# cmavro/GNN-RAG

Measured on NVIDIA H100. Metric: questions/sec (GNN forward+score) on WebQSP-shape subgraphs; agg-kernel HBM GB/s, higher is better.
Workload: dtype f32

## Files before the change

### gnn_rag_b200/csrc/linear_tc.cu

```cuda
#include "wgmma.cuh"

namespace gr {

int g_tc_cluster = 1;
int g_tc_bk = 32;
int g_tc_tma_store = 1;

namespace {

using namespace tc;
constexpr int kThreads = 384;
constexpr int kConsumerWarps = 8;
constexpr int kLaunchRegs = 168, kProducerRegs = 40, kConsumerRegs = 232;
static_assert(128 * kProducerRegs + 256 * kConsumerRegs <= kThreads * kLaunchRegs, "register budget");

__global__ void split_bf16_seg_kernel(const float* __restrict__ W, int64_t ldw, int64_t N, int64_t Kpad,
                                      int seg, int pitch, __nv_bfloat16* __restrict__ hi,
                                      __nv_bfloat16* __restrict__ lo, int64_t ldo) {
  const int64_t total = N * Kpad;
  const int64_t stride = (int64_t)gridDim.x * blockDim.x;
  for (int64_t i = (int64_t)blockIdx.x * blockDim.x + threadIdx.x; i < total; i += stride) {
    const int64_t n = i / Kpad, k = i - n * Kpad;
    const int sidx = (int)(k / pitch), c = (int)(k - (int64_t)sidx * pitch);
    float v = c < seg ? __ldg(W + n * ldw + (int64_t)sidx * seg + c) : 0.f;
    const __nv_bfloat16 h = __float2bfloat16_rn(v);
    hi[n * ldo + k] = h;
    lo[n * ldo + k] = __float2bfloat16_rn(v - __bfloat162float(h));
  }
}

__global__ void split_bf16_kernel(const float* __restrict__ A, int64_t lda, int64_t M, int64_t K,
                                  __nv_bfloat16* __restrict__ hi, __nv_bfloat16* __restrict__ lo,
                                  int64_t ldo, int vec_ok, int vec_st) {
  const int64_t kq = (K + 3) / 4;
  const int64_t total = M * kq;
  const int64_t stride = (int64_t)gridDim.x * blockDim.x;
  for (int64_t i = (int64_t)blockIdx.x * blockDim.x + threadIdx.x; i < total; i += stride) {
    const int64_t m = i / kq, k = (i - m * kq) * 4;
    float v[4] = {0.f, 0.f, 0.f, 0.f};
    const float* src = A + m * lda + k;
    if (vec_ok && k + 3 < K) {
      float4 t = __ldg(reinterpret_cast<const float4*>(src));
      v[0] = t.x; v[1] = t.y; v[2] = t.z; v[3] = t.w;
    } else {
#pragma unroll
      for (int q = 0; q < 4; ++q)
        if (k + q < K) v[q] = __ldg(src + q);
    }
    __nv_bfloat16 h[4], l[4];
#pragma unroll
    for (int q = 0; q < 4; ++q) {
      h[q] = __float2bfloat16_rn(v[q]);
      l[q] = __float2bfloat16_rn(v[q] - __bfloat162float(h[q]));
    }
    __nv_bfloat16* ph = hi + m * ldo + k;
    __nv_bfloat16* pl = lo + m * ldo + k;
    if (vec_st && k + 3 < ldo) {
      *reinterpret_cast<uint2*>(ph) = *reinterpret_cast<uint2*>(h);
      *reinterpret_cast<uint2*>(pl) = *reinterpret_cast<uint2*>(l);
    } else {
#pragma unroll
      for (int q = 0; q < 4; ++q)
        if (k + q < ldo) { ph[q] = h[q]; pl[q] = l[q]; }
    }
  }
}

struct TcParams {
  const float* bias;
  float* C;
  int64_t ldc;
  __nv_bfloat16* c_hi;
  __nv_bfloat16* c_lo;
  int64_t ldc16;
  const float* w_score;
  float* dots;
  int M, N, K, n_pad, n16, stages, num_tiles;
  uint32_t flags;
  int tma_store;
  int kg_T, kg_G, kg_pitch, kg_nkb, kg_one0, kg_one1, kg_nb0;
};

template <int NP, int CS, int BK, bool GROUPED>
__global__ void __launch_bounds__(kThreads, 1)
linear_tc_kernel(const __grid_constant__ CUtensorMap map_a_hi, const __grid_constant__ CUtensorMap map_a_lo,
                 const __grid_constant__ CUtensorMap map_w_hi, const __grid_constant__ CUtensorMap map_w_lo,
                 const __grid_constant__ CUtensorMap map_c, const __grid_constant__ CUtensorMap map_c_hi,
                 const __grid_constant__ CUtensorMap map_c_lo, const TcParams p) {
  extern __shared__ __align__(1024) uint8_t smem_raw[];
  uint8_t* smem = reinterpret_cast<uint8_t*>((reinterpret_cast<uintptr_t>(smem_raw) + 1023) & ~(uintptr_t)1023);
  const int a_bytes = BM * BK * 2;
  constexpr int w_bytes = NP * BK * 2;
  const bool single = (p.flags & GR_LINEAR_BF16_SINGLE) != 0;
  const int w_off = single ? a_bytes : 2 * a_bytes;
  const int stage_bytes = single ? a_bytes + w_bytes : 2 * a_bytes + 2 * w_bytes;
  uint8_t* s_out = smem + (size_t)p.stages * stage_bytes;
  uint64_t* bars = reinterpret_cast<uint64_t*>(s_out + 2 * kStageOutBytes);
  uint64_t* full_bar = bars;
  uint64_t* empty_bar = bars + p.stages;
  float* s_bias = reinterpret_cast<float*>(bars + 2 * p.stages);
  float* s_ws = s_bias + 256;
  for (int i = threadIdx.x; i < 256; i += kThreads) {
    s_bias[i] = (p.bias && i < p.N) ? p.bias[i] : 0.f;
    s_ws[i] = (p.w_score && i < p.N) ? p.w_score[i] : 0.f;
  }

  const int warp = threadIdx.x >> 5, lane = threadIdx.x & 31;
  const int nkb = GROUPED ? p.kg_nkb : (p.K + BK - 1) / BK;
  const int crank = CS > 1 ? (int)cluster_ctarank() : 0;
  const int ncluster = gridDim.x / CS, cid = blockIdx.x / CS;
  const int ngroups = (p.num_tiles + CS - 1) / CS;
  constexpr uint16_t kMask = (uint16_t)((1u << CS) - 1);

  if (threadIdx.x == 0) {
    for (int s = 0; s < p.stages; ++s) {
      mbar_init(&full_bar[s], 1);
      mbar_init(&empty_bar[s], kConsumerWarps * CS);
    }
    asm volatile("fence.mbarrier_init.release.cluster;" ::: "memory");
  }
  __syncthreads();
  if (CS > 1) cluster_sync_all();

  if (warp < 4) {
    asm volatile("setmaxnreg.dec.sync.aligned.u32 %0;" ::"n"(kProducerRegs));
    if (warp == 0 && lane == 0) {
      uint32_t phase = 0;
      int s = 0;
      constexpr int w_rows = NP / CS;
      const int w_slice = w_rows * BK * 2;
      for (int g = cid; g < ngroups; g += ncluster) {
        const int m0 = (g * CS + crank) * BM;
        for (int kb = 0; kb < nkb; ++kb) {
          mbar_wait(&empty_bar[s], phase ^ 1);
          uint8_t* st = smem + (size_t)s * stage_bytes;
          mbar_expect_tx(&full_bar[s], (uint32_t)stage_bytes);
          int a_col = kb * BK;
          if constexpr (GROUPED) {
            if (p.kg_nb0 == 0) {
              const int g = kb / p.kg_T, t = kb - g * p.kg_T, ni = p.kg_T >> 1;
              const int seg = t == 0 ? 0 : 1 + 2 * ((t - 1) % ni) + (t - 1) / ni;
              a_col = seg * p.kg_pitch + g * BK;
            } else {
              const int g = min(kb / p.kg_T, p.kg_G), t = kb - g * p.kg_T;
              a_col = t == 0 ? g * BK : p.kg_nb0 + (kb - g - 1) * BK;
            }
          }
          tma_load_2d(st, &map_a_hi, &full_bar[s], a_col, m0);
          if (!single) tma_load_2d(st + a_bytes, &map_a_lo, &full_bar[s], a_col, m0);
          if (CS == 1) {
            tma_load_2d(st + w_off, &map_w_hi, &full_bar[s], kb * BK, 0);
            if (!single) tma_load_2d(st + w_off + w_bytes, &map_w_lo, &full_bar[s], kb * BK, 0);
          } else {
            tma_load_2d_mc(st + w_off + crank * w_slice, &map_w_hi, &full_bar[s], kb * BK,
                           crank * w_rows, kMask);
            if (!single)
              tma_load_2d_mc(st + w_off + w_bytes + crank * w_slice, &map_w_lo, &full_bar[s], kb * BK,
                             crank * w_rows, kMask);
          }
          if (++s == p.stages) { s = 0; phase ^= 1; }
        }
      }
    }
  } else {
    asm volatile("setmaxnreg.inc.sync.aligned.u32 %0;" ::"n"(kConsumerRegs));
    const int cw = (warp - 4) >> 2, wq = warp & 3;
    const EpiOut e{s_bias, s_ws, (p.flags & GR_LINEAR_RELU) != 0};
    const int r = wq * 16 + (lane >> 2), cq = lane & 3;
    uint8_t* stg = s_out + (size_t)cw * kStageOutBytes;
    const bool issuer = wq == 0 && lane == 0;
    const bool vec_c = p.C && (p.ldc % 2 == 0) && ((reinterpret_cast<uintptr_t>(p.C) & 7) == 0);
    const bool vec_h = p.c_hi && (p.ldc16 % 2 == 0) && ((reinterpret_cast<uintptr_t>(p.c_hi) & 3) == 0) &&
                       ((reinterpret_cast<uintptr_t>(p.c_lo) & 3) == 0);
    uint32_t phase = 0;
    int s = 0;
    for (int g = cid; g < ngroups; g += ncluster) {
      const int tile = g * CS + crank;
      float acc[NP / 2];
#pragma unroll
      for (int i = 0; i < NP / 2; ++i) acc[i] = 0.f;
      int prev = -1;
      for (int kb = 0; kb < nkb; ++kb) {
        mbar_wait(&full_bar[s], phase);
        const uint32_t sa = smem_u32(smem + (size_t)s * stage_bytes);
        const uint32_t a_row = (uint32_t)(cw * WG_M * BK * 2);
        const uint64_t da_hi = make_smem_desc<BK>(sa + a_row), da_lo = make_smem_desc<BK>(sa + a_bytes + a_row);
        const uint64_t dw_hi = make_smem_desc<BK>(sa + w_off), dw_lo = make_smem_desc<BK>(sa + w_off + w_bytes);
        if constexpr (GROUPED) {
          if (kb >= p.kg_one0 && kb < p.kg_one1) mma_kblock<NP, BK, 1, false>(acc, da_hi, da_lo, dw_hi, dw_lo);
          else mma_kblock<NP, BK, BK / MMA_K, false>(acc, da_hi, da_lo, dw_hi, dw_lo);
        } else if (single) {
          mma_kblock<NP, BK, BK / MMA_K, true>(acc, da_hi, da_lo, dw_hi, dw_lo);
        } else {
          mma_kblock<NP, BK, BK / MMA_K, false>(acc, da_hi, da_lo, dw_hi, dw_lo);
        }
        wgmma_wait<1>();
        if (prev >= 0 && lane == 0) release_slot<CS>(&empty_bar[prev]);
        prev = s;
        if (++s == p.stages) { s = 0; phase ^= 1; }
      }
      wgmma_wait<0>();
      if (prev >= 0 && lane == 0) release_slot<CS>(&empty_bar[prev]);

      const int64_t row0 = (int64_t)tile * BM + cw * WG_M + r;
      float dot0 = 0.f, dot1 = 0.f;
#pragma unroll
      for (int q = 0; q < NP / 16; ++q) {
        const int c0 = 16 * q;
        if (c0 >= p.n_pad) continue;
        float v[8];
        epi_values(acc, q, cq, e, v, dot0, dot1);
        if (p.tma_store) {
          epi_store_tma(v, stg, r, cq, issuer, 1 + cw, &map_c, &map_c_hi, &map_c_lo, p.C != nullptr,
                        p.c_hi != nullptr, c0, tile * BM + cw * WG_M);
          continue;
        }
#pragma unroll
        for (int b = 0; b < 2; ++b) {
          const int col = c0 + 8 * b + 2 * cq;
#pragma unroll
          for (int hr = 0; hr < 2; ++hr) {
            const int64_t row = row0 + 8 * hr;
            if (row >= p.M) continue;
            const float x0 = v[4 * b + 2 * hr], x1 = v[4 * b + 2 * hr + 1];
            if (p.C) {
              float* c = p.C + row * p.ldc + col;
              if (vec_c && col + 1 < p.N) {
                *reinterpret_cast<float2*>(c) = make_float2(x0, x1);
              } else {
                if (col < p.N) c[0] = x0;
                if (col + 1 < p.N) c[1] = x1;
              }
            }
            if (p.c_hi) {
              uint32_t lo;
              const uint32_t hi = split_hi_lo(x0, x1, lo);
              unsigned short* ph = reinterpret_cast<unsigned short*>(p.c_hi + row * p.ldc16 + col);
              unsigned short* pl = reinterpret_cast<unsigned short*>(p.c_lo + row * p.ldc16 + col);
              if (vec_h && col + 1 < p.n16) {
                *reinterpret_cast<uint32_t*>(ph) = hi;
                *reinterpret_cast<uint32_t*>(pl) = lo;
              } else {
                if (col < p.n16) { ph[0] = (unsigned short)(hi & 0xFFFF); pl[0] = (unsigned short)(lo & 0xFFFF); }
                if (col + 1 < p.n16) { ph[1] = (unsigned short)(hi >> 16); pl[1] = (unsigned short)(lo >> 16); }
              }
            }
          }
        }
      }
      epi_dots(dot0, dot1, p.dots, row0, p.M, cq);
    }
    if (p.tma_store && issuer) asm volatile("cp.async.bulk.wait_group 0;" ::: "memory");
  }
  __syncthreads();
  if (CS > 1) cluster_sync_all();
}

struct TcPlan {
  int64_t kp;
  int n_pad, np, stages, bk;
  size_t a_plane_bytes, w_plane_bytes, total_bytes, w_only_bytes, smem_bytes;
  bool ok;
};

TcPlan plan_tc(int64_t M, int64_t N, int64_t K, bool single = false) {
  TcPlan t{};
  const int BK = g_tc_bk == 64 ? 64 : 32;
  t.ok = (N >= 8 && N <= 256 && K >= 8 && M >= 1);
  t.kp = (K + 7) / 8 * 8;
  t.n_pad = (int)((N + 15) / 16 * 16);
  t.np = t.n_pad <= 64 ? 64 : t.n_pad <= 128 ? 128 : t.n_pad <= 208 ? 208 : 256;
  const size_t stage = (single ? 1 : 2) * ((size_t)BM * BK * 2 + (size_t)t.np * BK * 2);
  int stages = (int)((227 * 1024 - 1024 - 2048 - 128 - 2 * kStageOutBytes) / stage);
  t.stages = stages > 8 ? 8 : stages;
  if (t.stages < 2) t.ok = false;
  t.bk = BK;
  t.smem_bytes = (size_t)t.stages * stage + 1024  + 2 * t.stages * 8 + 2 * 256 * 4 + 2 * kStageOutBytes;
  t.a_plane_bytes = align_up((size_t)M * t.kp * 2, 256);
  t.w_plane_bytes = align_up((size_t)N * t.kp * 2, 256);
  t.total_bytes = 2 * t.a_plane_bytes + 2 * t.w_plane_bytes;
  t.w_only_bytes = 2 * t.w_plane_bytes;
  return t;
}


int split_launch(const float* A, int64_t lda, int64_t M, int64_t K, __nv_bfloat16* hi, __nv_bfloat16* lo,
                 int64_t ldo, cudaStream_t stream) {
  int va = (lda % 4 == 0) && ((reinterpret_cast<uintptr_t>(A) & 15) == 0);
  int64_t work = M * ((K + 3) / 4);
  int grid = (int)std::min<int64_t>(ceil_div(work, 256), 32LL * sm_count());
  int vs = (ldo % 4 == 0) && ((reinterpret_cast<uintptr_t>(hi) & 7) == 0) &&
           ((reinterpret_cast<uintptr_t>(lo) & 7) == 0);
  split_bf16_kernel<<<grid, 256, 0, stream>>>(A, lda, M, K, hi, lo, ldo, va, vs);
  GR_CHECK_LAUNCH();
  return GR_OK;
}

template <int NP, int CS, int BK, bool GROUPED = false>
int launch_tc_cs(const CUtensorMap& m_a_hi, const CUtensorMap& m_a_lo, const CUtensorMap& m_w_hi,
                 const CUtensorMap& m_w_lo, const CUtensorMap& m_c, const CUtensorMap& m_c_hi,
                 const CUtensorMap& m_c_lo, const TcPlan& t, const TcParams& p, cudaStream_t stream) {
  const int ngroups = (p.num_tiles + CS - 1) / CS;
  const int nclusters = std::max(1, std::min(ngroups, sm_count() / CS));
  return launch_cluster<linear_tc_kernel<NP, CS, BK, GROUPED>>("gr_linear_tc", kLaunchRegs, CS, nclusters * CS, kThreads,
                                                               t.smem_bytes, stream, m_a_hi, m_a_lo, m_w_hi, m_w_lo,
                                                               m_c, m_c_hi, m_c_lo, p);
}

template <int NP>
int launch_tc_np(const CUtensorMap* const (&m)[7], int cs, const TcPlan& t, const TcParams& p, cudaStream_t stream) {
  if (p.kg_T) {
    if (cs == 2) return launch_tc_cs<NP, 2, 32, true>(*m[0], *m[1], *m[2], *m[3], *m[4], *m[5], *m[6], t, p, stream);
    return launch_tc_cs<NP, 1, 32, true>(*m[0], *m[1], *m[2], *m[3], *m[4], *m[5], *m[6], t, p, stream);
  }
  if (t.bk == 64) {
    if (cs == 2) return launch_tc_cs<NP, 2, 64>(*m[0], *m[1], *m[2], *m[3], *m[4], *m[5], *m[6], t, p, stream);
    return launch_tc_cs<NP, 1, 64>(*m[0], *m[1], *m[2], *m[3], *m[4], *m[5], *m[6], t, p, stream);
  }
  if (cs == 2) return launch_tc_cs<NP, 2, 32>(*m[0], *m[1], *m[2], *m[3], *m[4], *m[5], *m[6], t, p, stream);
  return launch_tc_cs<NP, 1, 32>(*m[0], *m[1], *m[2], *m[3], *m[4], *m[5], *m[6], t, p, stream);
}

int launch_tc(const __nv_bfloat16* a_hi, const __nv_bfloat16* a_lo, int64_t lda16,
              const __nv_bfloat16* w_hi, const __nv_bfloat16* w_lo, int64_t ldw16, const TcPlan& t,
              TcParams p, cudaStream_t stream) {
  p.n_pad = t.n_pad; p.stages = t.stages;
  p.num_tiles = (int)ceil_div(p.M, BM);
  int cs = (g_tc_cluster >= 2 && (t.np / 2) % 8 == 0 && p.num_tiles >= 2) ? 2 : 1;
  CUtensorMap m_a_hi, m_a_lo, m_w_hi, m_w_lo;
  const int64_t w_cols = p.kg_T ? ldw16 : p.K;
  const int64_t a_cols = p.kg_nb0 ? p.kg_nb0 + (int64_t)(p.kg_T - 1) * p.kg_pitch : p.K;
  if (!make_tmap(&m_a_hi, a_hi, p.M, a_cols, lda16, BM, t.bk) || !make_tmap(&m_a_lo, a_lo, p.M, a_cols, lda16, BM, t.bk) ||
      !make_tmap(&m_w_hi, w_hi, p.N, w_cols, ldw16, t.np / cs, t.bk) ||
      !make_tmap(&m_w_lo, w_lo, p.N, w_cols, ldw16, t.np / cs, t.bk)) {
    set_error("gr_linear_tc: cuTensorMapEncodeTiled failed (pointers must be 16-byte aligned, row strides "
              "multiples of 8 elements)");
    return GR_ERR_CUDA;
  }
  p.n16 = (int)std::min<int64_t>((p.N + 15) / 16 * 16, p.ldc16);
  CUtensorMap m_c, m_c_hi, m_c_lo;
  memset(&m_c, 0, sizeof(m_c)); memset(&m_c_hi, 0, sizeof(m_c_hi)); memset(&m_c_lo, 0, sizeof(m_c_lo));
  bool ok = g_tc_tma_store != 0;
  if (ok && p.C) ok = p.N % 4 == 0 && make_out_tmap(&m_c, p.C, p.M, p.N, p.ldc, 4);
  if (ok && p.c_hi) ok = make_out_tmap(&m_c_hi, p.c_hi, p.M, p.n16, p.ldc16, 2) &&
                         make_out_tmap(&m_c_lo, p.c_lo, p.M, p.n16, p.ldc16, 2);
  p.tma_store = ok ? 1 : 0;
  const CUtensorMap* m[7] = {&m_a_hi, &m_a_lo, &m_w_hi, &m_w_lo, &m_c, &m_c_hi, &m_c_lo};
  switch (t.np) {
    case 64: return launch_tc_np<64>(m, cs, t, p, stream);
    case 128: return launch_tc_np<128>(m, cs, t, p, stream);
    case 208: return launch_tc_np<208>(m, cs, t, p, stream);
    default: return launch_tc_np<256>(m, cs, t, p, stream);
  }
}

}

bool linear_tc_supported(int64_t M, int64_t N, int64_t K) {
  return plan_tc(M, N, K).ok && get_encode_fn() != nullptr;
}

}

extern "C" size_t gr_linear_tc_workspace_bytes(int64_t M, int64_t N, int64_t K) {
  if (M <= 0 || N <= 0 || K <= 0) return 0;
  return gr::plan_tc(M, N, K).total_bytes;
}

extern "C" size_t gr_linear_tc_planes_workspace_bytes(int64_t N, int64_t K) {
  if (N <= 0 || K <= 0) return 0;
  return gr::plan_tc(1, N, K).w_only_bytes;
}

extern "C" int gr_split_bf16(const float* A, int64_t lda, int64_t M, int64_t K, void* hi, void* lo,
                             int64_t ld_out, void* stream_) {
  using namespace gr;
  GR_CHECK_ARG(A && hi && lo, "null pointer");
  GR_CHECK_ARG(M > 0 && K > 0 && lda >= K && ld_out >= K && ld_out % 8 == 0, "bad shape / ld_out % 8 != 0");
  return split_launch(A, lda, M, K, reinterpret_cast<__nv_bfloat16*>(hi), reinterpret_cast<__nv_bfloat16*>(lo),
                      ld_out, reinterpret_cast<cudaStream_t>(stream_));
}

extern "C" int gr_linear_tc(const float* A, int64_t lda, const float* W, int64_t ldw, const float* bias,
                            float* C, int64_t ldc, int64_t M, int64_t N, int64_t K, uint32_t flags,
                            void* workspace, size_t workspace_bytes, void* stream_) {
  using namespace gr;
  cudaStream_t stream = reinterpret_cast<cudaStream_t>(stream_);
  GR_CHECK_ARG(A && W && C && workspace, "null pointer");
  GR_CHECK_ARG(M > 0 && N > 0 && K > 0, "M, N, K must be positive");
  GR_CHECK_ARG(lda >= K && ldw >= K && ldc >= N, "leading dimension smaller than row length");
  GR_CHECK_ARG(M < (int64_t)0x7fffffff - BM, "M exceeds int32 range");
  TcPlan t = plan_tc(M, N, K);
  if (!t.ok) {
    set_error("gr_linear_tc: unsupported shape M=%lld N=%lld K=%lld (need 8 <= N <= 256, K >= 8)",
              (long long)M, (long long)N, (long long)K);
    return GR_ERR_UNSUPPORTED;
  }
  if (int rc = check_workspace(__func__, workspace, workspace_bytes, t.total_bytes)) return rc;
  if ((reinterpret_cast<uintptr_t>(workspace) & 255) != 0) {
    set_error("gr_linear_tc: workspace must be 256-byte aligned");
    return GR_ERR_INVALID_ARG;
  }
  char* ws = reinterpret_cast<char*>(workspace);
  __nv_bfloat16* a_hi = reinterpret_cast<__nv_bfloat16*>(ws);
  __nv_bfloat16* a_lo = reinterpret_cast<__nv_bfloat16*>(ws + t.a_plane_bytes);
  __nv_bfloat16* w_hi = reinterpret_cast<__nv_bfloat16*>(ws + 2 * t.a_plane_bytes);
  __nv_bfloat16* w_lo = reinterpret_cast<__nv_bfloat16*>(ws + 2 * t.a_plane_bytes + t.w_plane_bytes);
  int rc = split_launch(A, lda, M, K, a_hi, a_lo, t.kp, stream);
  if (rc != GR_OK) return rc;
  rc = split_launch(W, ldw, N, K, w_hi, w_lo, t.kp, stream);
  if (rc != GR_OK) return rc;
  TcParams p{};
  p.bias = bias; p.C = C; p.ldc = ldc;
  p.M = (int)M; p.N = (int)N; p.K = (int)K; p.flags = flags;
  return launch_tc(a_hi, a_lo, t.kp, w_hi, w_lo, t.kp, t, p, stream);
}

extern "C" int gr_linear_tc_planes(const void* A_hi, const void* A_lo, int64_t lda16, const float* W,
                                   int64_t ldw, const float* bias, float* C, int64_t ldc, void* C_hi,
                                   void* C_lo, int64_t ldc16, const float* w_score, float* dots, int64_t M,
                                   int64_t N, int64_t K, int64_t k_seg, int64_t k_seg_pitch, uint32_t flags,
                                   void* workspace, size_t workspace_bytes, void* stream_) {
  using namespace gr;
  cudaStream_t stream = reinterpret_cast<cudaStream_t>(stream_);
  GR_CHECK_ARG(A_hi && (A_lo || (flags & GR_LINEAR_BF16_SINGLE)) && W && workspace, "null pointer");
  GR_CHECK_ARG(C || C_hi, "no output requested");
  GR_CHECK_ARG(M > 0 && N > 0 && K > 0, "M, N, K must be positive");
  const bool grouped = (flags & GR_LINEAR_K_GROUPED) != 0;
  const bool korder = (flags & GR_LINEAR_K_ORDER_PLANES) != 0;
  GR_CHECK_ARG(!korder || grouped, "GR_LINEAR_K_ORDER_PLANES modifies GR_LINEAR_K_GROUPED and needs it");
  if (grouped) {
    GR_CHECK_ARG(k_seg > 0 && k_seg_pitch >= k_seg && k_seg_pitch % 16 == 0,
                 "GR_LINEAR_K_GROUPED needs segmented K: k_seg > 0 and k_seg_pitch >= k_seg, a multiple of 16");
    GR_CHECK_ARG(K % k_seg_pitch == 0 && (K / k_seg_pitch) % 2 == 1,
                 "GR_LINEAR_K_GROUPED needs an odd number of segments (2 I + 1)");
    GR_CHECK_ARG(g_tc_bk != 64, "GR_LINEAR_K_GROUPED needs 32-column k-blocks (tc_bk = 32)");
    GR_CHECK_ARG(!(flags & GR_LINEAR_BF16_SINGLE), "GR_LINEAR_K_GROUPED does not combine with GR_LINEAR_BF16_SINGLE");
  }
  const bool segmented = grouped || (k_seg > 0 && k_seg_pitch > k_seg);
  GR_CHECK_ARG(lda16 >= K && lda16 % 8 == 0, "lda16 must be >= K and a multiple of 8");
  GR_CHECK_ARG(!segmented || K % k_seg_pitch == 0, "K must be a multiple of k_seg_pitch");
  GR_CHECK_ARG(ldw >= (segmented ? K / k_seg_pitch * k_seg : K), "ldw smaller than the weight row length");
  GR_CHECK_ARG(!C || ldc >= N, "ldc smaller than N");
  GR_CHECK_ARG(!C_hi || (C_lo && ldc16 >= N), "C_lo missing or ldc16 smaller than N");
  GR_CHECK_ARG(!dots || w_score, "dots requested without w_score");
  GR_CHECK_ARG(M < (int64_t)0x7fffffff - BM, "M exceeds int32 range");
  TcPlan t = plan_tc(M, N, K, (flags & GR_LINEAR_BF16_SINGLE) != 0);
  if (!t.ok) {
    set_error("gr_linear_tc_planes: unsupported shape M=%lld N=%lld K=%lld", (long long)M, (long long)N,
              (long long)K);
    return GR_ERR_UNSUPPORTED;
  }
  const int num_ins = grouped ? (int)(K / k_seg_pitch / 2) : 0;
  const GroupedK gk = grouped ? plan_grouped_k(k_seg_pitch, num_ins, N, korder) : GroupedK{};
  const int64_t nb0 = (k_seg_pitch + 31) / 32 * 32;
  GR_CHECK_ARG(!korder || lda16 >= nb0 + 2 * num_ins * k_seg_pitch,
               "GR_LINEAR_K_ORDER_PLANES: lda16 must cover the neighbour region (round32(k_seg_pitch) + (K - k_seg_pitch) "
               "columns)");
  const size_t w_plane_bytes = grouped ? gk.w_plane_bytes : t.w_plane_bytes;
  if (workspace_bytes < 2 * w_plane_bytes || (reinterpret_cast<uintptr_t>(workspace) & 255) != 0) {
    set_error("gr_linear_tc_planes: workspace too small or not 256-byte aligned");
    return GR_ERR_WORKSPACE;
  }
  char* ws = reinterpret_cast<char*>(workspace);
  __nv_bfloat16* w_hi = reinterpret_cast<__nv_bfloat16*>(ws);
  __nv_bfloat16* w_lo = reinterpret_cast<__nv_bfloat16*>(ws + w_plane_bytes);
  int rc = GR_OK;
  if (flags & GR_LINEAR_W_PRESPLIT) {
  } else if (grouped) {
    rc = grouped_w_split(W, ldw, N, (int)k_seg, num_ins, gk, w_hi, w_lo, stream);
  } else if (segmented) {
    int64_t work = N * K;
    int grid = (int)std::min<int64_t>(ceil_div(work, 256), 32LL * sm_count());
    split_bf16_seg_kernel<<<grid, 256, 0, stream>>>(W, ldw, N, K, (int)k_seg, (int)k_seg_pitch, w_hi, w_lo, t.kp);
    GR_CHECK_LAUNCH();
  } else {
    rc = split_launch(W, ldw, N, K, w_hi, w_lo, t.kp, stream);
  }
  if (rc != GR_OK) return rc;
  TcParams p{};
  p.bias = bias; p.C = C; p.ldc = ldc;
  p.c_hi = reinterpret_cast<__nv_bfloat16*>(C_hi); p.c_lo = reinterpret_cast<__nv_bfloat16*>(C_lo);
  p.ldc16 = ldc16; p.w_score = w_score; p.dots = dots;
  p.M = (int)M; p.N = (int)N; p.K = (int)K; p.flags = flags;
  if (grouped) {
    p.kg_T = 2 * num_ins + 1; p.kg_pitch = (int)k_seg_pitch; p.kg_nkb = gk.nkb;
    const bool tail = gk.ksteps_last == 1;
    if (!korder) {
      p.kg_G = gk.G;
      p.kg_one0 = tail ? (gk.G - 1) * p.kg_T : gk.nkb; p.kg_one1 = gk.nkb;
    } else {
      p.kg_G = tail ? gk.G - 1 : gk.G; p.kg_nb0 = (int)nb0;
      p.kg_one0 = tail ? p.kg_G * p.kg_T : gk.nkb; p.kg_one1 = tail ? p.kg_one0 + 1 : gk.nkb;
    }
  }
  return launch_tc(reinterpret_cast<const __nv_bfloat16*>(A_hi),
                   reinterpret_cast<const __nv_bfloat16*>(A_lo ? A_lo : A_hi), lda16, w_hi, w_lo,
                   grouped ? gk.kp : t.kp, t, p, stream);
}
```

### gnn_rag_b200/csrc/wgmma.cuh

```cuda
#pragma once
#include <cuda.h>
#include <cuda_bf16.h>

#include "common.cuh"

namespace gr {
namespace tc {

constexpr int BM = 128;
constexpr int WG_M = 64;
constexpr int MMA_K = 16;

struct GroupedK {
  int G, ksteps_last, nkb;
  int64_t kp;
  size_t w_plane_bytes;
};
GroupedK plan_grouped_k(int64_t pitch, int I, int64_t N_out, bool packed = false);
int grouped_w_split(const float* W, int64_t ldw, int64_t N_out, int D, int I, const GroupedK& k, __nv_bfloat16* hi,
                    __nv_bfloat16* lo, cudaStream_t stream);

typedef CUresult (*EncodeTiledFn)(CUtensorMap*, CUtensorMapDataType, cuuint32_t, void*, const cuuint64_t*,
                                  const cuuint64_t*, const cuuint32_t*, const cuuint32_t*,
                                  CUtensorMapInterleave, CUtensorMapSwizzle, CUtensorMapL2promotion,
// ... 166 lines not shown
  } else if constexpr (N == 32) {
    GR_WGMMA(32, GR_REGS16, 16, 17, GR_ACC8(0), GR_ACC8(8));
  } else if constexpr (N == 64) {
    GR_WGMMA(64, GR_REGS32, 32, 33, GR_ACC32(0));
  } else if constexpr (N == 128) {
    GR_WGMMA(128, GR_REGS64, 64, 65, GR_ACC32(0), GR_ACC32(32));
  } else if constexpr (N == 208) {
    GR_WGMMA(208, GR_REGS104, 104, 105, GR_ACC32(0), GR_ACC32(32), GR_ACC32(64), GR_ACC8(96));
  } else {
    static_assert(N == 256, "instruction widths: 16, 32, 64, 128, 208, 256");
    GR_WGMMA(256, GR_REGS128, 128, 129, GR_ACC32(0), GR_ACC32(32), GR_ACC32(64), GR_ACC32(96));
  }
}
#undef GR_WGMMA
#undef GR_REGS128
#undef GR_REGS104
#undef GR_REGS64
#undef GR_REGS32
#undef GR_REGS16
#undef GR_REGS8
#undef GR_ACC32
#undef GR_ACC8

template <int NP, int NI, int BK, int C0 = 0>
__device__ __forceinline__ void wgmma_product(float (&acc)[NP / 2], uint64_t a, uint64_t b) {
  constexpr int n = NP - C0 < NI ? NP - C0 : NI;
  wgmma_bf16<n, C0 / 2>(acc, a, b + (uint64_t)((C0 * BK * 2) >> 4));
  if constexpr (C0 + n < NP) wgmma_product<NP, NI, BK, C0 + n>(acc, a, b);
}

template <int NP, int BK, int KSTEPS, bool SINGLE, int NI = NP>
__device__ __forceinline__ void mma_kblock(float (&acc)[NP / 2], uint64_t da_hi, uint64_t da_lo, uint64_t dw_hi,
                                           uint64_t dw_lo) {
  static_assert(KSTEPS >= 1 && KSTEPS <= BK / MMA_K, "k-steps of one k-block");
  acc_fence(acc);
  wgmma_fence();
#pragma unroll
  for (int k = 0; k < KSTEPS; ++k) {
    const uint64_t adv = (uint64_t)((k * MMA_K * 2) >> 4);
    wgmma_product<NP, NI, BK>(acc, da_hi + adv, dw_hi + adv);
    if (!SINGLE) {
      wgmma_product<NP, NI, BK>(acc, da_hi + adv, dw_lo + adv);
      wgmma_product<NP, NI, BK>(acc, da_lo + adv, dw_hi + adv);
    }
  }
  wgmma_commit();
  acc_fence(acc);
}

struct EpiOut {
  const float* bias;
  const float* w_score;
  bool relu;
};

template <int R>
__device__ __forceinline__ void epi_values(const float (&a)[R], int q, int cq, const EpiOut& e, float (&v)[8],
                                           float& dot0, float& dot1) {
#pragma unroll
  for (int b = 0; b < 2; ++b) {
    const int col = 16 * q + 8 * b + 2 * cq;
    const float2 bb = *reinterpret_cast<const float2*>(e.bias + col);
    const float2 ww = *reinterpret_cast<const float2*>(e.w_score + col);
#pragma unroll
    for (int i = 0; i < 4; ++i) {
      float x = a[8 * q + 4 * b + i] + ((i & 1) ? bb.y : bb.x);
      if (e.relu) x = fmaxf(x, 0.f);
      v[4 * b + i] = x;
    }
    dot0 = fmaf(v[4 * b + 0], ww.x, dot0); dot0 = fmaf(v[4 * b + 1], ww.y, dot0);
    dot1 = fmaf(v[4 * b + 2], ww.x, dot1); dot1 = fmaf(v[4 * b + 3], ww.y, dot1);
  }
}

__device__ __forceinline__ uint32_t split_hi_lo(float x0, float x1, uint32_t& lo) {
  const __nv_bfloat162 h2 = __floats2bfloat162_rn(x0, x1);
  const float2 hf = __bfloat1622float2(h2);
  const __nv_bfloat162 l2 = __floats2bfloat162_rn(x0 - hf.x, x1 - hf.y);
  lo = *reinterpret_cast<const uint32_t*>(&l2);
  return *reinterpret_cast<const uint32_t*>(&h2);
}

constexpr int kStageOutBytes = WG_M * 16 * 4 + 2 * WG_M * 16 * 2;
__device__ __forceinline__ void epi_store_tma(const float (&v)[8], uint8_t* stg, int r, int cq, bool issuer,
                                              int bar_id, const CUtensorMap* map_c, const CUtensorMap* map_hi,
                                              const CUtensorMap* map_lo, bool has_c, bool has_planes, int c0, int m0) {
  if (issuer) asm volatile("cp.async.bulk.wait_group.read 0;" ::: "memory");
  named_bar_sync(bar_id, 128);
  float* s_c = reinterpret_cast<float*>(stg);
  uint32_t* s_h = reinterpret_cast<uint32_t*>(stg + WG_M * 16 * 4);
  uint32_t* s_l = reinterpret_cast<uint32_t*>(stg + WG_M * 16 * 4 + WG_M * 16 * 2);
#pragma unroll
  for (int b = 0; b < 2; ++b) {
    const int col = 8 * b + 2 * cq;
#pragma unroll
    for (int hr = 0; hr < 2; ++hr) {
      const int row = r + 8 * hr;
      const float x0 = v[4 * b + 2 * hr], x1 = v[4 * b + 2 * hr + 1];
      if (has_c) *reinterpret_cast<float2*>(s_c + row * 16 + col) = make_float2(x0, x1);
      if (has_planes) {
        uint32_t lo;
        const uint32_t hi = split_hi_lo(x0, x1, lo);
        s_h[row * 8 + col / 2] = hi;
        s_l[row * 8 + col / 2] = lo;
      }
    }
  }
  asm volatile("fence.proxy.async.shared::cta;" ::: "memory");
  named_bar_sync(bar_id, 128);
  if (issuer) {
    if (has_c) tma_store_2d(map_c, stg, c0, m0);
    if (has_planes) {
      tma_store_2d(map_hi, stg + WG_M * 16 * 4, c0, m0);
      tma_store_2d(map_lo, stg + WG_M * 16 * 4 + WG_M * 16 * 2, c0, m0);
    }
    asm volatile("cp.async.bulk.commit_group;" ::: "memory");
  }
}

__device__ __forceinline__ void epi_dots(float dot0, float dot1, float* dots, int64_t row0, int64_t M, int cq) {
  dot0 += __shfl_xor_sync(0xffffffffu, dot0, 1);
  dot0 += __shfl_xor_sync(0xffffffffu, dot0, 2);
  dot1 += __shfl_xor_sync(0xffffffffu, dot1, 1);
  dot1 += __shfl_xor_sync(0xffffffffu, dot1, 2);
  if (dots && cq == 0) {
    if (row0 < M) { dots[row0] = dot0; dots[M + row0] = 0.f; }
    if (row0 + 8 < M) { dots[row0 + 8] = dot1; dots[M + row0 + 8] = 0.f; }
  }
}

template <auto Kernel, typename... Args>
int launch_cluster(const char* fn, int launch_regs, int cs, int grid, int threads, size_t smem, cudaStream_t stream,
                   const Args&... args) {
  if (int rc = opt_in_smem<Kernel>(fn, 227 * 1024)) return rc;
  static int num_regs = 0;
  if (num_regs == 0) {
    cudaFuncAttributes fa{};
    GR_CHECK_CUDA_AS(fn, cudaFuncGetAttributes(&fa, Kernel));
    num_regs = fa.numRegs;
  }
  if (num_regs != launch_regs) {
    set_error("%s: kernel was compiled with %d registers per thread, the warpgroup budget needs %d", fn, num_regs,
              launch_regs);
    return GR_ERR_UNSUPPORTED;
  }
  cudaLaunchConfig_t cfg{};
  cfg.gridDim = dim3((unsigned)grid);
  cfg.blockDim = dim3((unsigned)threads);
  cfg.dynamicSmemBytes = smem;
  cfg.stream = stream;
  cudaLaunchAttribute attr[1];
  attr[0].id = cudaLaunchAttributeClusterDimension;
  attr[0].val.clusterDim.x = cs;
  attr[0].val.clusterDim.y = 1;
  attr[0].val.clusterDim.z = 1;
  cfg.attrs = attr;
  cfg.numAttrs = 1;
  GR_CHECK_CUDA_AS(fn, cudaLaunchKernelEx(&cfg, Kernel, args...));
  return GR_OK;
}

}
}
```

### include/gnnrag_b200.h

```cpp
#ifndef GNNRAG_B200_H_
#define GNNRAG_B200_H_

#include <stddef.h>
#include <stdint.h>

#ifdef __cplusplus
extern "C" {
#endif

#define GR_ABI_VERSION 1

typedef enum gr_status {
  GR_OK = 0,
  GR_ERR_INVALID_ARG = -1,
  GR_ERR_CUDA = -2,
  GR_ERR_WORKSPACE = -3,
  GR_ERR_UNSUPPORTED = -4
} gr_status;

#define GR_LINEAR_RELU 1u
#define GR_LINEAR_EXACT_FP32 2u
#define GR_LINEAR_BF16_SINGLE 8u
#define GR_LINEAR_W_PRESPLIT 4u

#define GR_LINEAR_K_GROUPED 16u
#define GR_LINEAR_K_ORDER_PLANES 32u

int gr_abi_version(void);
const char* gr_last_error(void);
int gr_set_option(const char* name, int64_t value);
static inline int64_t gr_pad4(int64_t n) { return (n + 3) & ~(int64_t)3; }

size_t gr_csr_build_workspace_bytes(int64_t F, int64_t Nt);
int gr_csr_build(const void* heads, const void* rels, const void* tails, int idx_bytes,
                 int64_t F, int64_t Nt, int64_t num_rel_rows,
                 int32_t* rowptr_t, int32_t* src_t, int32_t* rel_t, int32_t* fact_t,
                 int32_t* rowptr_h, int32_t* src_h, int32_t* rel_h, int32_t* fact_h,
                 int32_t* status, const int32_t* nfacts, void* workspace, size_t workspace_bytes, void* stream);

int gr_gather_f32(const float* in, const int32_t* fact, float* out, int64_t F, void* stream);

int gr_linear(const float* A, int64_t lda, const float* W, int64_t ldw, const float* bias,
              const float* addend, int64_t ld_addend, int64_t addend_rows,
              float* C, int64_t ldc, int64_t M, int64_t N, int64_t K, uint32_t flags, void* stream);

size_t gr_linear_tc_workspace_bytes(int64_t M, int64_t N, int64_t K);
int gr_linear_tc(const float* A, int64_t lda, const float* W, int64_t ldw, const float* bias,
                 float* C, int64_t ldc, int64_t M, int64_t N, int64_t K, uint32_t flags,
                 void* workspace, size_t workspace_bytes, void* stream);
size_t gr_linear_tc_planes_workspace_bytes(int64_t N, int64_t K);
int gr_linear_tc_planes(const void* A_hi, const void* A_lo, int64_t lda16, const float* W, int64_t ldw,
                        const float* bias, float* C, int64_t ldc, void* C_hi, void* C_lo, int64_t ldc16,
                        const float* w_score, float* dots, int64_t M, int64_t N, int64_t K,
                        int64_t k_seg, int64_t k_seg_pitch,
                        uint32_t flags, void* workspace, size_t workspace_bytes, void* stream);
int gr_split_bf16(const float* A, int64_t lda, int64_t M, int64_t K, void* hi, void* lo, int64_t ld_out,
                  void* stream);

int gr_aggregate(const int32_t* rowptr, const int32_t* src, const int32_t* rel, const float* w,
                 const float* prior, const float* table, const float* ins,
                 float* out, int64_t out_row_stride, int64_t out_col0, int64_t seg_stride,
                 float* possible, int B, int N, int D, int I, int64_t F, void* stream);

int gr_aggregate_backward(const int32_t* rowptr, const int32_t* src, const int32_t* rel, const float* w,
                          const float* prior, const float* table, const float* ins, const float* grad_out,
                          int64_t grad_row_stride, int64_t grad_col0, int64_t seg_stride, float* grad_table,
                          float* grad_ins, float* grad_prior, int B, int N, int D, int I, int64_t F, void* stream);

int gr_aggregate_dual(const int32_t* rowptr_t, const int32_t* src_t, const int32_t* rel_t,
                      const float* w_t, const int32_t* rowptr_h, const int32_t* src_h,
                      const int32_t* rel_h, const float* w_h, const float* prior,
                      const float* table_fwd, const float* table_inv, const float* ins,
                      float* out, int64_t out_row_stride, int64_t out_col0, int64_t seg_pitch,
                      void* out_hi, void* out_lo, int64_t ld_planes,
                      int B, int N, int D, int I, int64_t F, void* stream);

int gr_pad_table256(const float* table, int64_t ldt, int64_t rows, int D, float* pn, void* stream);
int gr_aggregate_dual_abs_supported(int N, int D, int64_t seg_pitch, int64_t R1);
int gr_aggregate_dual_abs(const int32_t* rowptr_t, const int32_t* src_t, const int32_t* rel_t, const float* w_t,
                         const int32_t* rowptr_h, const int32_t* src_h, const int32_t* rel_h, const float* w_h,
                         const float* prior, const float* pn_fwd, const float* pn_inv, int64_t table_rows,
                         const float* ins, void* out_hi, void* out_lo, int64_t ld_planes, int64_t out_col0,
                         int64_t seg_pitch, int B, int N, int D, int I, int64_t F, int32_t* tile_counter, void* stream);
#define GR_AGG_K_ORDER 1u
int gr_aggregate_dual_abs_ex(const int32_t* rowptr_t, const int32_t* src_t, const int32_t* rel_t, const float* w_t,
                             const int32_t* rowptr_h, const int32_t* src_h, const int32_t* rel_h, const float* w_h,
                             const float* prior, const float* pn_fwd, const float* pn_inv, int64_t table_rows,
                             const float* ins, void* out_hi, void* out_lo, int64_t ld_planes, int64_t out_col0,
                             int64_t seg_pitch, int B, int N, int D, int I, int64_t F, int32_t* tile_counter,
                             uint32_t flags, void* stream);

int gr_fused_profile_read(unsigned long long* out, int n);
int gr_fused_layer_supported(int64_t N_nodes, int64_t D, int64_t seg_pitch, int I, int64_t N_out);
size_t gr_fused_layer_workspace_bytes(int64_t D, int64_t seg_pitch, int I, int64_t N_out);
size_t gr_fused_ell_bytes(int B, int N_nodes, int64_t F);
int gr_fused_ell_build(const int32_t* rowptr_t, const int32_t* src_t, const int32_t* rel_t, const float* w_t,
                       const int32_t* rowptr_h, const int32_t* src_h, const int32_t* rel_h, const float* w_h,
                       int B, int N_nodes, int64_t F, void* ell, size_t ell_bytes, void* stream);
int gr_fused_layer(const int32_t* rowptr_t, const int32_t* src_t, const int32_t* rel_t, const float* w_t,
                   const int32_t* rowptr_h, const int32_t* src_h, const int32_t* rel_h, const float* w_h,
                   const float* prior, const float* pn_fwd, const float* pn_inv, const float* ins,
                   const void* h_hi, const void* h_lo, int64_t ldh16, int64_t seg_pitch, const float* W,
                   int64_t ldw, const float* bias, float* C, int64_t ldc, void* C_hi, void* C_lo,
                   int64_t ldc16, const float* w_score, float* dots, int B, int N_nodes, int D, int I,
                   int64_t N_out, int64_t F, uint32_t flags, void* workspace, size_t workspace_bytes,
                   void* ell, size_t ell_bytes, void* stream);

int gr_debug_store_probe(void* hi, void* lo, int64_t Nt, int64_t ld, int col_start, int ncols, int mode,
                         void* stream);

int gr_type_layer(const int32_t* rowptr_t, const int32_t* rel_t, const float* w_t,
                  const int32_t* rowptr_h, const int32_t* rel_h, const float* w_h,
                  const float* table, float* out, int64_t out_row_stride,
                  void* out_hi, void* out_lo, int64_t ld_planes,
                  int B, int N, int D, int64_t F, void* stream);

size_t gr_graft_stage_workspace_bytes(int64_t B, int64_t max_fact);
int gr_graft_stage(const int64_t* e2f_b, const int64_t* e2f_f, const int64_t* e2f_e, int64_t F_e2f,
                   const int64_t* f2e_b, const int64_t* f2e_e, const int64_t* f2e_f, int64_t F_f2e,
                   const int64_t* kb_fact_rel, int B, int N, int64_t max_fact, int64_t R1, int32_t* heads,
                   int32_t* rels, int32_t* tails, int32_t* slot_of, int32_t* nfacts, int32_t* status,
                   const int32_t* live, void* workspace, size_t workspace_bytes, void* stream);
int gr_graft_attention(const float* qh, const float* qmask, int Q, const float* rel, int64_t ldr, int64_t R1,
                       const int64_t* kb_fact_rel, int B, int64_t max_fact, int D, const int32_t* rowptr_h,
                       const int32_t* fact_h, const int32_t* slot_of, int N, float* W, float* Wt, float* E,
                       int32_t* status, void* stream);
int gr_graft_aggregate(const int32_t* rowptr_t, const int32_t* src_t, const int32_t* rel_t, const int32_t* fact_t,
                       const int32_t* slot_of, const float* Wt, const float* E, const float* prior,
                       const float* self_tab, int64_t ld_self, const float* head_tab, int64_t ld_head,
                       const float* q2e, double lambda, float* sum_out, int64_t ld_sum, void* out_hi, void* out_lo,
                       int64_t ld_planes, int64_t col_sum, int64_t col_indeg, int64_t col_q2e, float* indeg_out,
                       float* prior_next, int B, int N, int D, void* stream);

// ... 255 lines not shown
```

Baseline: 13020.

## Add triple-buffered TMA store ring to linear epilogue and shrink plane-only staging

Measured after the change: 13180 (median of 6 runs). 1.3% higher.

```diff
diff --git a/gnn_rag_b200/csrc/linear_tc.cu b/gnn_rag_b200/csrc/linear_tc.cu
--- a/gnn_rag_b200/csrc/linear_tc.cu
+++ b/gnn_rag_b200/csrc/linear_tc.cu
@@ -78,6 +78,8 @@
   int M, N, K, n_pad, n16, stages, num_tiles;
   uint32_t flags;
   int tma_store;
+  int epi_ring;
+  int stg_bytes;
   int kg_T, kg_G, kg_pitch, kg_nkb, kg_one0, kg_one1, kg_nb0;
 };
 
@@ -95,7 +97,7 @@
   const int w_off = single ? a_bytes : 2 * a_bytes;
   const int stage_bytes = single ? a_bytes + w_bytes : 2 * a_bytes + 2 * w_bytes;
   uint8_t* s_out = smem + (size_t)p.stages * stage_bytes;
-  uint64_t* bars = reinterpret_cast<uint64_t*>(s_out + 2 * kStageOutBytes);
+  uint64_t* bars = reinterpret_cast<uint64_t*>(s_out + (size_t)2 * p.epi_ring * p.stg_bytes);
   uint64_t* full_bar = bars;
   uint64_t* empty_bar = bars + p.stages;
   float* s_bias = reinterpret_cast<float*>(bars + 2 * p.stages);
@@ -167,7 +169,10 @@
     const int cw = (warp - 4) >> 2, wq = warp & 3;
     const EpiOut e{s_bias, s_ws, (p.flags & GR_LINEAR_RELU) != 0};
     const int r = wq * 16 + (lane >> 2), cq = lane & 3;
-    uint8_t* stg = s_out + (size_t)cw * kStageOutBytes;
+    uint8_t* stg = s_out + (size_t)cw * p.epi_ring * p.stg_bytes;
+    const int po = p.C ? WG_M * 16 * 4 : 0;
+    const bool ring = p.epi_ring == kEpiRing;
+    int slot = 0;
     const bool issuer = wq == 0 && lane == 0;
     const bool vec_c = p.C && (p.ldc % 2 == 0) && ((reinterpret_cast<uintptr_t>(p.C) & 7) == 0);
     const bool vec_h = p.c_hi && (p.ldc16 % 2 == 0) && ((reinterpret_cast<uintptr_t>(p.c_hi) & 3) == 0) &&
@@ -211,8 +216,14 @@
         float v[8];
         epi_values(acc, q, cq, e, v, dot0, dot1);
         if (p.tma_store) {
-          epi_store_tma(v, stg, r, cq, issuer, 1 + cw, &map_c, &map_c_hi, &map_c_lo, p.C != nullptr,
-                        p.c_hi != nullptr, c0, tile * BM + cw * WG_M);
+          if (ring) {
+            epi_store_tma_ring(v, stg, slot, r, cq, issuer, 1 + cw, &map_c, &map_c_hi, &map_c_lo, p.C != nullptr,
+                               p.c_hi != nullptr, c0, tile * BM + cw * WG_M);
+            if (++slot == kEpiRing) slot = 0;
+          } else {
+            epi_store_tma(v, stg, r, cq, issuer, 1 + cw, &map_c, &map_c_hi, &map_c_lo, p.C != nullptr,
+                          p.c_hi != nullptr, c0, tile * BM + cw * WG_M, po);
+          }
           continue;
         }
 #pragma unroll
@@ -259,11 +270,15 @@
 struct TcPlan {
   int64_t kp;
   int n_pad, np, stages, bk;
+  int epi_ring;
+  int stg_bytes;
   size_t a_plane_bytes, w_plane_bytes, total_bytes, w_only_bytes, smem_bytes;
   bool ok;
 };
 
-TcPlan plan_tc(int64_t M, int64_t N, int64_t K, bool single = false) {
+constexpr size_t kSmemLimit = 227 * 1024;
+
+TcPlan plan_tc(int64_t M, int64_t N, int64_t K, bool single = false, bool with_c = true) {
   TcPlan t{};
   const int BK = g_tc_bk == 64 ? 64 : 32;
   t.ok = (N >= 8 && N <= 256 && K >= 8 && M >= 1);
@@ -271,11 +286,15 @@
   t.n_pad = (int)((N + 15) / 16 * 16);
   t.np = t.n_pad <= 64 ? 64 : t.n_pad <= 128 ? 128 : t.n_pad <= 208 ? 208 : 256;
   const size_t stage = (single ? 1 : 2) * ((size_t)BM * BK * 2 + (size_t)t.np * BK * 2);
-  int stages = (int)((227 * 1024 - 1024 - 2048 - 128 - 2 * kStageOutBytes) / stage);
+  t.stg_bytes = with_c ? kStageOutBytes : kStagePlanesBytes;
+  int stages = (int)((kSmemLimit - 1024 - 2048 - 128 - 2 * t.stg_bytes) / stage);
   t.stages = stages > 8 ? 8 : stages;
   if (t.stages < 2) t.ok = false;
   t.bk = BK;
-  t.smem_bytes = (size_t)t.stages * stage + 1024  + 2 * t.stages * 8 + 2 * 256 * 4 + 2 * kStageOutBytes;
+  t.smem_bytes = (size_t)t.stages * stage + 1024  + 2 * t.stages * 8 + 2 * 256 * 4 + 2 * t.stg_bytes;
+  const size_t ring_extra = 2 * (size_t)(kEpiRing - 1) * kStageOutBytes;
+  t.epi_ring = with_c && !single && t.smem_bytes + ring_extra <= kSmemLimit ? kEpiRing : 1;
+  if (t.epi_ring > 1) t.smem_bytes += ring_extra;
   t.a_plane_bytes = align_up((size_t)M * t.kp * 2, 256);
   t.w_plane_bytes = align_up((size_t)N * t.kp * 2, 256);
   t.total_bytes = 2 * t.a_plane_bytes + 2 * t.w_plane_bytes;
@@ -324,7 +343,7 @@
 int launch_tc(const __nv_bfloat16* a_hi, const __nv_bfloat16* a_lo, int64_t lda16,
               const __nv_bfloat16* w_hi, const __nv_bfloat16* w_lo, int64_t ldw16, const TcPlan& t,
               TcParams p, cudaStream_t stream) {
-  p.n_pad = t.n_pad; p.stages = t.stages;
+  p.n_pad = t.n_pad; p.stages = t.stages; p.epi_ring = t.epi_ring; p.stg_bytes = t.stg_bytes;
   p.num_tiles = (int)ceil_div(p.M, BM);
   int cs = (g_tc_cluster >= 2 && (t.np / 2) % 8 == 0 && p.num_tiles >= 2) ? 2 : 1;
   CUtensorMap m_a_hi, m_a_lo, m_w_hi, m_w_lo;
@@ -340,7 +359,7 @@
   p.n16 = (int)std::min<int64_t>((p.N + 15) / 16 * 16, p.ldc16);
   CUtensorMap m_c, m_c_hi, m_c_lo;
   memset(&m_c, 0, sizeof(m_c)); memset(&m_c_hi, 0, sizeof(m_c_hi)); memset(&m_c_lo, 0, sizeof(m_c_lo));
-  bool ok = g_tc_tma_store != 0;
+  bool ok = g_tc_tma_store != 0 && (p.C || p.c_hi);
   if (ok && p.C) ok = p.N % 4 == 0 && make_out_tmap(&m_c, p.C, p.M, p.N, p.ldc, 4);
   if (ok && p.c_hi) ok = make_out_tmap(&m_c_hi, p.c_hi, p.M, p.n16, p.ldc16, 2) &&
                          make_out_tmap(&m_c_lo, p.c_lo, p.M, p.n16, p.ldc16, 2);
@@ -370,6 +389,19 @@
 extern "C" size_t gr_linear_tc_planes_workspace_bytes(int64_t N, int64_t K) {
   if (N <= 0 || K <= 0) return 0;
   return gr::plan_tc(1, N, K).w_only_bytes;
+}
+
+extern "C" int gr_linear_tc_plan(int64_t N, int64_t K, uint32_t flags, int with_c, int* stages, int* epi_ring,
+                                 size_t* smem_bytes) {
+  using namespace gr;
+  GR_CHECK_ARG(stages && epi_ring && smem_bytes, "null pointer");
+  const TcPlan t = plan_tc(1, N, K, (flags & GR_LINEAR_BF16_SINGLE) != 0, with_c != 0);
+  if (!t.ok) {
+    set_error("gr_linear_tc_plan: unsupported shape N=%lld K=%lld", (long long)N, (long long)K);
+    return GR_ERR_UNSUPPORTED;
+  }
+  *stages = t.stages; *epi_ring = t.epi_ring; *smem_bytes = t.smem_bytes;
+  return GR_OK;
 }
 
 extern "C" int gr_split_bf16(const float* A, int64_t lda, int64_t M, int64_t K, void* hi, void* lo,
@@ -424,7 +456,7 @@
   using namespace gr;
   cudaStream_t stream = reinterpret_cast<cudaStream_t>(stream_);
   GR_CHECK_ARG(A_hi && (A_lo || (flags & GR_LINEAR_BF16_SINGLE)) && W && workspace, "null pointer");
-  GR_CHECK_ARG(C || C_hi, "no output requested");
+  GR_CHECK_ARG(C || C_hi || dots, "no output requested");
   GR_CHECK_ARG(M > 0 && N > 0 && K > 0, "M, N, K must be positive");
   const bool grouped = (flags & GR_LINEAR_K_GROUPED) != 0;
   const bool korder = (flags & GR_LINEAR_K_ORDER_PLANES) != 0;
@@ -445,7 +477,7 @@
   GR_CHECK_ARG(!C_hi || (C_lo && ldc16 >= N), "C_lo missing or ldc16 smaller than N");
   GR_CHECK_ARG(!dots || w_score, "dots requested without w_score");
   GR_CHECK_ARG(M < (int64_t)0x7fffffff - BM, "M exceeds int32 range");
-  TcPlan t = plan_tc(M, N, K, (flags & GR_LINEAR_BF16_SINGLE) != 0);
+  TcPlan t = plan_tc(M, N, K, (flags & GR_LINEAR_BF16_SINGLE) != 0, C != nullptr);
   if (!t.ok) {
     set_error("gr_linear_tc_planes: unsupported shape M=%lld N=%lld K=%lld", (long long)M, (long long)N,
               (long long)K);
diff --git a/gnn_rag_b200/csrc/wgmma.cuh b/gnn_rag_b200/csrc/wgmma.cuh
--- a/gnn_rag_b200/csrc/wgmma.cuh
+++ b/gnn_rag_b200/csrc/wgmma.cuh
@@ -272,14 +272,12 @@
 }
 
 constexpr int kStageOutBytes = WG_M * 16 * 4 + 2 * WG_M * 16 * 2;
-__device__ __forceinline__ void epi_store_tma(const float (&v)[8], uint8_t* stg, int r, int cq, bool issuer,
-                                              int bar_id, const CUtensorMap* map_c, const CUtensorMap* map_hi,
-                                              const CUtensorMap* map_lo, bool has_c, bool has_planes, int c0, int m0) {
-  if (issuer) asm volatile("cp.async.bulk.wait_group.read 0;" ::: "memory");
-  named_bar_sync(bar_id, 128);
+constexpr int kStagePlanesBytes = 2 * WG_M * 16 * 2;
+__device__ __forceinline__ void epi_stage_chunk(const float (&v)[8], uint8_t* stg, int po, int r, int cq, bool has_c,
+                                                bool has_planes) {
   float* s_c = reinterpret_cast<float*>(stg);
-  uint32_t* s_h = reinterpret_cast<uint32_t*>(stg + WG_M * 16 * 4);
-  uint32_t* s_l = reinterpret_cast<uint32_t*>(stg + WG_M * 16 * 4 + WG_M * 16 * 2);
+  uint32_t* s_h = reinterpret_cast<uint32_t*>(stg + po);
+  uint32_t* s_l = reinterpret_cast<uint32_t*>(stg + po + WG_M * 16 * 2);
 #pragma unroll
   for (int b = 0; b < 2; ++b) {
     const int col = 8 * b + 2 * cq;
@@ -296,16 +294,42 @@
       }
     }
   }
+}
+__device__ __forceinline__ void epi_issue_chunk(const uint8_t* stg, int po, const CUtensorMap* map_c,
+                                                const CUtensorMap* map_hi, const CUtensorMap* map_lo, bool has_c,
+                                                bool has_planes, int c0, int m0) {
+  if (has_c) tma_store_2d(map_c, stg, c0, m0);
+  if (has_planes) {
+    tma_store_2d(map_hi, stg + po, c0, m0);
+    tma_store_2d(map_lo, stg + po + WG_M * 16 * 2, c0, m0);
+  }
+  asm volatile("cp.async.bulk.commit_group;" ::: "memory");
+}
+
+__device__ __forceinline__ void epi_store_tma(const float (&v)[8], uint8_t* stg, int r, int cq, bool issuer,
+                                              int bar_id, const CUtensorMap* map_c, const CUtensorMap* map_hi,
+                                              const CUtensorMap* map_lo, bool has_c, bool has_planes, int c0, int m0,
+                                              int po = WG_M * 16 * 4) {
+  if (issuer) asm volatile("cp.async.bulk.wait_group.read 0;" ::: "memory");
+  named_bar_sync(bar_id, 128);
+  epi_stage_chunk(v, stg, po, r, cq, has_c, has_planes);
   asm volatile("fence.proxy.async.shared::cta;" ::: "memory");
   named_bar_sync(bar_id, 128);
-  if (issuer) {
-    if (has_c) tma_store_2d(map_c, stg, c0, m0);
-    if (has_planes) {
-      tma_store_2d(map_hi, stg + WG_M * 16 * 4, c0, m0);
-      tma_store_2d(map_lo, stg + WG_M * 16 * 4 + WG_M * 16 * 2, c0, m0);
-    }
-    asm volatile("cp.async.bulk.commit_group;" ::: "memory");
-  }
+  if (issuer) epi_issue_chunk(stg, po, map_c, map_hi, map_lo, has_c, has_planes, c0, m0);
+}
+
+constexpr int kEpiRing = 3;
+__device__ __forceinline__ void epi_store_tma_ring(const float (&v)[8], uint8_t* ring, int slot, int r, int cq,
+                                                   bool issuer, int bar_id, const CUtensorMap* map_c,
+                                                   const CUtensorMap* map_hi, const CUtensorMap* map_lo, bool has_c,
+                                                   bool has_planes, int c0, int m0) {
+  static_assert(kEpiRing == 3, "the wait below leaves kEpiRing - 2 = 1 group reading");
+  uint8_t* stg = ring + (size_t)slot * kStageOutBytes;
+  epi_stage_chunk(v, stg, WG_M * 16 * 4, r, cq, has_c, has_planes);
+  asm volatile("fence.proxy.async.shared::cta;" ::: "memory");
+  if (issuer) asm volatile("cp.async.bulk.wait_group.read 1;" ::: "memory");
+  named_bar_sync(bar_id, 128);
+  if (issuer) epi_issue_chunk(stg, WG_M * 16 * 4, map_c, map_hi, map_lo, has_c, has_planes, c0, m0);
 }
 
 __device__ __forceinline__ void epi_dots(float dot0, float dot1, float* dots, int64_t row0, int64_t M, int cq) {
diff --git a/include/gnnrag_b200.h b/include/gnnrag_b200.h
--- a/include/gnnrag_b200.h
+++ b/include/gnnrag_b200.h
@@ -49,6 +49,8 @@
                  float* C, int64_t ldc, int64_t M, int64_t N, int64_t K, uint32_t flags,
                  void* workspace, size_t workspace_bytes, void* stream);
 size_t gr_linear_tc_planes_workspace_bytes(int64_t N, int64_t K);
+int gr_linear_tc_plan(int64_t N, int64_t K, uint32_t flags, int with_c, int* stages, int* epi_ring,
+                      size_t* smem_bytes);
 int gr_linear_tc_planes(const void* A_hi, const void* A_lo, int64_t lda16, const float* W, int64_t ldw,
                         const float* bias, float* C, int64_t ldc, void* C_hi, void* C_lo, int64_t ldc16,
                         const float* w_score, float* dots, int64_t M, int64_t N, int64_t K,
```
